# piljoong-jeong/nerf_meets_mlx

Measured on AMD Instinct MI355X. Metric: train+render rays/sec on Lego 800x800 (synthetic), coarse+fine 64+128, higher is better.
Workload: dtype split16 (fp16x2 render / bf16x2 train MFMA operands ~ 22 / 16 significand bits; fp32 accumulate)

## Files before the change

### nerf_meets_mlx_amd/csrc/mlp22.h

```cpp
#pragma once
#include <hip/hip_runtime.h>
#include <stdint.h>

namespace nerf {
namespace f22 {

constexpr int F_PAIRS = 1172, F_FRAGS = 2 * F_PAIRS, F_PADDED = 2368, BIAS_FLOATS = 2496;
constexpr int64_t PACKED_BYTES = (int64_t)F_PADDED * 1024 + (int64_t)BIAS_FLOATS * 4;

extern int g_tiles;
int pack(const float* params, void* packed22, hipStream_t s);
int forward(const void* packed22, const float* x, const float* rays, const float* z, int64_t M, int n, int freq_mode,
            float* out, int persistent_wgs, hipStream_t s);

}
}
```

### nerf_meets_mlx_amd/csrc/mlp22.hip

```cpp
#include "mlp_layout.h"
#include "mlp22.h"

#ifndef NERF_F22_SINF
#define NERF_F22_SINF 0
#endif

#ifndef NERF_F22_PIN
#define NERF_F22_PIN 1
#endif
#ifndef NERF_F22_AGPR
#define NERF_F22_AGPR 1
#endif
#ifndef NERF_F22_MIXSUB
#define NERF_F22_MIXSUB 1
#endif
#ifndef NERF_F22_RG3
#define NERF_F22_RG3 4
#endif
#ifndef NERF_F22_IGLP
#define NERF_F22_IGLP 0
#endif

namespace nerf {
namespace f22 {

typedef _Float16 h8 __attribute__((ext_vector_type(8)));
typedef _Float16 h2 __attribute__((ext_vector_type(2)));
typedef float f32x2 __attribute__((ext_vector_type(2)));
typedef unsigned int u32x4 __attribute__((ext_vector_type(4)));

constexpr float LO_SCALE = 2048.0f, LO_INV = 1.0f / 2048.0f;
constexpr float F16_MIN_NORMAL = 6.103515625e-05f;
constexpr int CHUNKS = F_PADDED / RING_CHUNK;
static_assert(CHUNKS * RING_CHUNK == F_PADDED && F_FRAGS % 4 == 0 && F_PAIRS == L::F16_TOTAL, "f22 stream layout");

struct HiLo { unsigned hi, lo; };
__device__ __forceinline__ HiLo split2(float v0, float v1) {
  const f32x2 v = {v0, v1};
  const h2 hh = __builtin_convertvector(v, h2);
#if NERF_F22_MIXSUB
  const f32x2 r = {__builtin_fmaf((float)hh[0], -LO_SCALE, v0 * LO_SCALE), __builtin_fmaf((float)hh[1], -LO_SCALE, v1 * LO_SCALE)};
#else
  const f32x2 r = {(v0 - (float)hh[0]) * LO_SCALE, (v1 - (float)hh[1]) * LO_SCALE};
#endif
  return HiLo{__builtin_bit_cast(unsigned, hh), __builtin_bit_cast(unsigned, __builtin_convertvector(r, h2))};
}

constexpr int PACK_THREADS = (F_PADDED / 2) * 64 + BIAS_FLOATS;
__global__ void __launch_bounds__(256) pack22_kernel(const float* __restrict__ p, u32x4* __restrict__ wf,
                                                     float* __restrict__ bias) {
  const int t = blockIdx.x * 256 + threadIdx.x;
  if (t < (F_PADDED / 2) * 64) {
    const int fp = t >> 6, lane = t & 63;
    u32x4 hi = {0u, 0u, 0u, 0u}, lo = {0u, 0u, 0u, 0u};
    if (fp < F_PAIRS) {
#pragma unroll
      for (int j = 0; j < 8; j += 2) {
        float w[2];
        _Float16 wh[2], wl[2];
#pragma unroll
        for (int e = 0; e < 2; ++e) {
          w[e] = fwd_src16(p, fp, lane & 15, lane >> 4, j + e);
          wh[e] = __builtin_fabsf(w[e]) < F16_MIN_NORMAL ? (_Float16)0.0f : (_Float16)w[e];
          wl[e] = (_Float16)((w[e] - (float)wh[e]) * LO_SCALE);
        }
        const h2 a = {wh[0], wh[1]}, b = {wl[0], wl[1]};
        hi[j >> 1] = __builtin_bit_cast(unsigned, a);
        lo[j >> 1] = __builtin_bit_cast(unsigned, b);
      }
    }
    wf[(2 * fp) * 64 + lane] = hi;
    wf[(2 * fp + 1) * 64 + lane] = lo;
  } else if (t < PACK_THREADS) {
    const int s = t - (F_PADDED / 2) * 64;
    float v = 0.0f;
    if (s < 2048) v = p[L::pb(s >> 8) + (s & 255)];
    else if (s < L::BI_ALPHA) v = p[L::P_BF + (s - L::BI_FEAT)];
    else if (s < L::BI_DIR) v = (s == L::BI_ALPHA) ? p[L::P_BA] : 0.0f;
    else if (s < L::BI_RGB) v = p[L::P_BD + (s - L::BI_DIR)];
    else v = (s - L::BI_RGB) < 3 ? p[L::P_BR + (s - L::BI_RGB)] : 0.0f;
    bias[s] = v;
  }
}

__device__ __forceinline__ float sin_acc(float x, float f, float ph) {
  const float a = x * f;
#if NERF_F22_SINF
  return ph != 0.0f ? cosf(a) : sinf(a);
#else
  const float k = __builtin_rintf(a * 0.15915494309189535f);
  float r = __builtin_fmaf(-k, 6.2831854820251465f, a);
  r = __builtin_fmaf(-k, -1.7484556000744487e-07f, r);
  return __builtin_amdgcn_sinf(__builtin_fmaf(r, 0.15915494309189535f, ph));
#endif
}

struct Pe22 { float fa, fb, fc, phc, fd; int g; };
__device__ __forceinline__ Pe22 pe22_setup(const PeFreq& fr, int g) {
  Pe22 q;
  q.fa = g == 0 ? fr.pos[0] : g == 1 ? fr.pos[2] : g == 2 ? fr.pos[4] : fr.pos[6];
  q.fb = g == 0 ? fr.pos[1] : g == 1 ? fr.pos[3] : g == 2 ? fr.pos[5] : fr.pos[7];
  q.fc = g < 2 ? fr.pos[8] : fr.pos[9];
  q.phc = (g & 1) ? 0.25f : 0.0f;
  q.fd = g == 0 ? fr.dir[0] : g == 1 ? fr.dir[1] : g == 2 ? fr.dir[2] : fr.dir[3];
  q.g = g;
  return q;
}

template <int COUNT>
__device__ __forceinline__ void split_slots(const float (&v)[COUNT], u32x4* hi, u32x4* lo) {
#pragma unroll
  for (int j = 0; j < COUNT; j += 2) {
    const HiLo q = split2(v[j], v[j + 1]);
    hi[j >> 3][(j & 7) >> 1] = q.hi; lo[j >> 3][(j & 7) >> 1] = q.lo;
  }
}

__device__ __forceinline__ void pe22_pos(const Pe22& q, const float (&p)[3], u32x4 (&peh)[2], u32x4 (&pel)[2]) {
  float v[16];
#pragma unroll
  for (int sl = 0; sl < 12; ++sl) v[sl] = sin_acc(p[sl % 3], sl < 6 ? q.fa : q.fb, (sl % 6) >= 3 ? 0.25f : 0.0f);
#pragma unroll
  for (int k = 0; k < 3; ++k) v[12 + k] = sin_acc(p[k], q.fc, q.phc);
  v[15] = q.g == 0 ? p[0] : q.g == 1 ? p[1] : q.g == 2 ? p[2] : 0.0f;
  split_slots<16>(v, peh, pel);
}
__device__ __forceinline__ void pe22_dir(const Pe22& q, const float (&d)[3], u32x4 (&dph)[1], u32x4 (&dpl)[1]) {
  float w[8];
#pragma unroll
  for (int j = 0; j < 6; ++j) w[j] = sin_acc(d[j % 3], q.fd, j >= 3 ? 0.25f : 0.0f);
  w[6] = q.g == 0 ? d[0] : q.g == 1 ? d[1] : q.g == 2 ? d[2] : 0.0f;
  w[7] = 0.0f;
  split_slots<8>(w, dph, dpl);
}
__device__ __forceinline__ void pe22_encode(const Pe22& q, const float (&p)[3], const float (&d)[3], u32x4 (&peh)[2],
                                            u32x4 (&pel)[2], u32x4 (&dph)[1], u32x4 (&dpl)[1]) {
  pe22_pos(q, p, peh, pel);
  pe22_dir(q, d, dph, dpl);
}
__device__ __forceinline__ void pe22_row(const float* __restrict__ row, int g, u32x4 (&peh)[2], u32x4 (&pel)[2],
                                         u32x4 (&dph)[1], u32x4 (&dpl)[1]) {
  float v[16], w[8];
#pragma unroll
  for (int sl = 0; sl < 16; ++sl) {
    const int ch = pos_chan16(sl >> 3, g, sl & 7);
    v[sl] = ch >= 0 ? row[ch] : 0.0f;
  }
#pragma unroll
  for (int j = 0; j < 8; ++j) {
    const int ch = dir_chan16(g, j);
    w[j] = ch >= 0 ? row[63 + ch] : 0.0f;
  }
  split_slots<16>(v, peh, pel);
  split_slots<8>(w, dph, dpl);
}

__device__ __forceinline__ f32x4 mfma16(const u32x4& a, const u32x4& b, const f32x4& c) {
#if NERF_ABLATE == 41 || NERF_ABLATE == 42
  return c;
#endif
  return __builtin_amdgcn_mfma_f32_16x16x32_f16(__builtin_bit_cast(h8, a), __builtin_bit_cast(h8, b), c, 0, 0, 0);
}

template <int NS, int KS, int NT, bool RELU, class WS, bool PARK_LDS = false>
__device__ __forceinline__ void layer22(WS& ws, int pbase, int bias_slot, const u32x4 (&ih)[NS][KS], const u32x4 (&il)[NS][KS],
                                        u32x4 (&oh)[NS][NT / 2], u32x4 (&ol)[NS][NT / 2], int lane, unsigned park_addr = 0u) {
  const int g = lane >> 4;
  f32x4 pm[NS], pc[NS];
  if (PARK_LDS) asm volatile("ds_write_b128 %0, %1" :: "v"(park_addr), "v"(il[NS - 1][KS - 1]) : "memory");
#if NERF_F22_IGLP >= 0
  __builtin_amdgcn_iglp_opt(NERF_F22_IGLP);
#endif
  constexpr int NP = 2 * NS;
  auto piece = [&](int nt, int pcs, f32x4 (&m)[NS], f32x4 (&c)[NS]) {
    const int s = pcs >> 1, i = 2 * (pcs & 1);
#if NERF_ABLATE == 41 || NERF_ABLATE == 42
    return;
#endif
#if NERF_F22_PIN
    if (pcs == 0) {
#pragma unroll
      for (int t = 0; t < NS; ++t) asm volatile("" : "+v"(m[t]), "+v"(c[t]));
    }
#endif
    float v0 = __builtin_fmaf(c[s][i], LO_INV, m[s][i]), v1 = __builtin_fmaf(c[s][i + 1], LO_INV, m[s][i + 1]);
    if (RELU) { v0 = __builtin_elementwise_maximum(v0, 0.0f); v1 = __builtin_elementwise_maximum(v1, 0.0f); }
    const HiLo q = split2(v0, v1);
    oh[s][nt >> 1][2 * (nt & 1) + (i >> 1)] = q.hi; ol[s][nt >> 1][2 * (nt & 1) + (i >> 1)] = q.lo;
#if NERF_F22_AGPR
    if ((nt & 1) && i == 2) asm volatile("" : "+a"(oh[s][nt >> 1]), "+a"(ol[s][nt >> 1]));
#endif
  };
  auto piece_at = [](int q) { return NS == 2 ? (KS >= 8 ? 1 + 2 * q : (q * KS) / 4) : (KS >= 8 ? 1 + (q * (KS - 1)) / NP : (q * KS) / NP); };
#pragma unroll
  for (int nt = 0; nt < NT; ++nt) {
    const float4 b = ws.bias4(bias_slot + 16 * nt + 4 * g);
    f32x4 m[NS], c[NS];
    m[0][0] = b.x; m[0][1] = b.y; m[0][2] = b.z; m[0][3] = b.w;
    c[0] = f32x4{0.0f, 0.0f, 0.0f, 0.0f};
#pragma unroll
    for (int t = 1; t < NS; ++t) { m[t] = m[0]; c[t] = c[0]; }
#pragma unroll
    for (int ks = 0; ks < KS; ++ks) {
      const int fp = pbase + nt * KS + ks;
      const u32x4 ah = __builtin_bit_cast(u32x4, next_frag(ws, 2 * fp, lane));
      const u32x4 al = __builtin_bit_cast(u32x4, next_frag(ws, 2 * fp + 1, lane));
      if (NS == 2) {
        m[0] = mfma16(ah, ih[0][ks], m[0]);
        c[0] = mfma16(ah, il[0][ks], c[0]);
        m[1] = mfma16(ah, ih[1][ks], m[1]);
        c[1] = mfma16(ah, il[1][ks], c[1]);
        c[0] = mfma16(al, ih[0][ks], c[0]);
        c[1] = mfma16(al, ih[1][ks], c[1]);
      } else {
#pragma unroll
        for (int t = 0; t < NS; ++t) {
          m[t] = mfma16(ah, ih[t][ks], m[t]);
          if (PARK_LDS && t == NS - 1 && ks == KS - 1) {
            u32x4 b;
            asm volatile("ds_read_b128 %0, %1\n\ts_waitcnt lgkmcnt(0)" : "=v"(b) : "v"(park_addr) : "memory");
            c[t] = mfma16(ah, b, c[t]);
          } else {
            c[t] = mfma16(ah, il[t][ks], c[t]);
          }
        }
#pragma unroll
        for (int t = 0; t < NS; ++t) c[t] = mfma16(al, ih[t][ks], c[t]);
      }
      if (nt > 0) {
#pragma unroll
        for (int q = 0; q < NP; ++q)
          if (piece_at(q) == ks) piece(nt - 1, q, pm, pc);
      }
    }
#pragma unroll
    for (int t = 0; t < NS; ++t) { pm[t] = m[t]; pc[t] = c[t]; }
  }
#pragma unroll
  for (int q = 0; q < NP; ++q) piece(NT - 1, q, pm, pc);
}

template <int NS, int KS, class WS>
__device__ __forceinline__ void head22(WS& ws, int pbase, int bias_slot, const u32x4 (&ih)[NS][KS], const u32x4 (&il)[NS][KS],
                                       f32x4 (&out)[NS], int lane) {
  const int g = lane >> 4;
  const float4 b = ws.bias4(bias_slot + 4 * g);
  f32x4 m[NS], c[NS];
  m[0][0] = b.x; m[0][1] = b.y; m[0][2] = b.z; m[0][3] = b.w;
  c[0] = f32x4{0.0f, 0.0f, 0.0f, 0.0f};
#pragma unroll
  for (int t = 1; t < NS; ++t) { m[t] = m[0]; c[t] = c[0]; }
#pragma unroll
  for (int ks = 0; ks < KS; ++ks) {
    const u32x4 ah = __builtin_bit_cast(u32x4, next_frag(ws, 2 * (pbase + ks), lane));
    const u32x4 al = __builtin_bit_cast(u32x4, next_frag(ws, 2 * (pbase + ks) + 1, lane));
    if (NS == 2) {
      m[0] = mfma16(ah, ih[0][ks], m[0]);
      c[0] = mfma16(ah, il[0][ks], c[0]);
      m[1] = mfma16(ah, ih[1][ks], m[1]);
      c[1] = mfma16(ah, il[1][ks], c[1]);
      c[0] = mfma16(al, ih[0][ks], c[0]);
      c[1] = mfma16(al, ih[1][ks], c[1]);
    } else {
#pragma unroll
      for (int t = 0; t < NS; ++t) { m[t] = mfma16(ah, ih[t][ks], m[t]); c[t] = mfma16(ah, il[t][ks], c[t]); }
#pragma unroll
      for (int t = 0; t < NS; ++t) c[t] = mfma16(al, ih[t][ks], c[t]);
    }
  }
#pragma unroll
  for (int s = 0; s < NS; ++s)
#pragma unroll
    for (int i = 0; i < 4; ++i) out[s][i] = __builtin_fmaf(c[s][i], LO_INV, m[s][i]);
}

constexpr int NW22 = 4, NW22_ = NW22;
constexpr int PARK_OFF = RING_LDS_BYTES;
template <int NS> constexpr int park_bytes() { return NS > 2 ? (6 * NS + 4) * 64 * NW22_ * 4 : 0; }
template <int K> __device__ __forceinline__ void lds_put(unsigned addr, float v) {
  asm volatile("ds_write_b32 %0, %1 offset:%2" :: "v"(addr), "v"(v), "i"(1024 * K) : "memory");
}
template <int K> __device__ __forceinline__ float lds_get(unsigned addr) {
  float v;
  asm volatile("ds_read_b32 %0, %1 offset:%2\n\ts_waitcnt lgkmcnt(0)" : "=v"(v) : "v"(addr), "i"(1024 * K) : "memory");
  return v;
}
template <int S> __device__ __forceinline__ void park_put(unsigned park, const float (&p)[3], const float (&d)[3]) {
  lds_put<6 * S + 0>(park, p[0]); lds_put<6 * S + 1>(park, p[1]); lds_put<6 * S + 2>(park, p[2]);
  lds_put<6 * S + 3>(park, d[0]); lds_put<6 * S + 4>(park, d[1]); lds_put<6 * S + 5>(park, d[2]);
}
template <int S, int OFF> __device__ __forceinline__ void park_get(unsigned park, float (&v)[3]) {
  v[0] = lds_get<6 * S + OFF>(park); v[1] = lds_get<6 * S + OFF + 1>(park); v[2] = lds_get<6 * S + OFF + 2>(park);
}
__device__ __forceinline__ void park_put_s(int s, unsigned park, const float (&p)[3], const float (&d)[3]) {
  if (s == 0) park_put<0>(park, p, d); else if (s == 1) park_put<1>(park, p, d); else park_put<2>(park, p, d);
}
template <int OFF> __device__ __forceinline__ void park_get_s(int s, unsigned park, float (&v)[3]) {
  if (s == 0) park_get<0, OFF>(park, v); else if (s == 1) park_get<1, OFF>(park, v); else park_get<2, OFF>(park, v);
}

template <int NS, int MODE, class WS>
__device__ __forceinline__ void tiles22(const FwdArgs& a, WS& ws, int64_t wtile0, int64_t nwtiles, int lane, PassQueue& pq) {
  constexpr bool RECOMP = NS > 2;
  static_assert(!RECOMP || MODE == 1, "the 48-sample form takes rays + depths");
  const int c = lane & 15, g = lane >> 4;
  u32x4 peh[NS][2], pel[NS][2], dph[NS][1], dpl[NS][1];
  const unsigned park = ws.lds0 + PARK_OFF + 4u * (unsigned)(ws.wv * 64 + lane);
  pq.ask(ws.wv, lane);
  const Pe22 q = pe22_setup(a.fr, g);
  {
    const int64_t wt = wtile0 < nwtiles ? wtile0 : nwtiles - 1;
#pragma unroll
    for (int s = 0; s < NS; ++s) {
      int64_t m = wt * (16 * NS) + 16 * s + c; if (m >= a.M) m = a.M - 1;
      if (MODE == 0) {
        pe22_row(a.x + m * 90, g, peh[s], pel[s], dph[s], dpl[s]);
      } else {
        const int64_t ray = (int64_t)((unsigned)m / (unsigned)a.n);
        const float* rr = a.rays + ray * NERF_RAY_STRIDE;
        float p[3], d[3];
#if NERF_ABLATE == 3
        (void)rr;
#pragma unroll
        for (int k = 0; k < 3; ++k) { p[k] = 0.001f * (float)(m & 1023) + (float)k; d[k] = 0.5f; }
#else
        const float zv = a.z[m];
#pragma unroll
        for (int k = 0; k < 3; ++k) { p[k] = rr[k] + zv * rr[3 + k]; d[k] = rr[8 + k]; }
#endif
        if (RECOMP) {
          park_put_s(s, park, p, d);
          pe22_pos(q, p, peh[s], pel[s]);
        } else {
          pe22_encode(q, p, d, peh[s], pel[s], dph[s], dpl[s]);
        }
      }
    }
  }
  pq.publish(ws.wv);
  u32x4 hah[NS][8], hal[NS][8], hbh[NS][8], hbl[NS][8];
  layer22<NS, 2, 16, true>(ws, L16::F_L0, 0, peh, pel, hah, hal, lane);
  layer22<NS, 8, 16, true>(ws, L16::F_L1 + 0 * 128, 256, hah, hal, hbh, hbl, lane);
  layer22<NS, 8, 16, true>(ws, L16::F_L1 + 1 * 128, 512, hbh, hbl, hah, hal, lane);
  layer22<NS, 8, 16, true>(ws, L16::F_L1 + 2 * 128, 768, hah, hal, hbh, hbl, lane);
  layer22<NS, 8, 16, true>(ws, L16::F_L1 + 3 * 128, 1024, hbh, hbl, hah, hal, lane);
  {
    u32x4 cth[NS][10], ctl[NS][10];
#pragma unroll
    for (int s = 0; s < NS; ++s) {
      if (RECOMP) {
        float pp[3];
        park_get_s<0>(s, park, pp);
        pe22_pos(q, pp, peh[s], pel[s]);
      }
      cth[s][0] = peh[s][0]; cth[s][1] = peh[s][1]; ctl[s][0] = pel[s][0]; ctl[s][1] = pel[s][1];
#pragma unroll
      for (int k = 0; k < 8; ++k) { cth[s][2 + k] = hah[s][k]; ctl[s][2 + k] = hal[s][k]; }
    }
    layer22<NS, 10, 16, true, WS, (NS > 2)>(ws, L16::F_L5, 1280, cth, ctl, hbh, hbl, lane,
                                            ws.lds0 + PARK_OFF + 6 * NS * 64 * NW22 * 4 + 16u * (unsigned)(ws.wv * 64 + lane));
  }
  layer22<NS, 8, 16, true>(ws, L16::F_L6, 1536, hbh, hbl, hah, hal, lane);
  layer22<NS, 8, 16, true>(ws, L16::F_L7, 1792, hah, hal, hbh, hbl, lane);
  layer22<NS, 8, 16, false>(ws, L16::F_FA, L::BI_FEAT, hbh, hbl, hah, hal, lane);
  f32x4 alpha[NS];
  head22<NS, 8>(ws, L16::F_FA + 128, L::BI_ALPHA, hbh, hbl, alpha, lane);
  u32x4 hdh[NS][4], hdl[NS][4];
  {
    u32x4 cth[NS][9], ctl[NS][9];
#pragma unroll
    for (int s = 0; s < NS; ++s) {
#pragma unroll
      for (int k = 0; k < 8; ++k) { cth[s][k] = hah[s][k]; ctl[s][k] = hal[s][k]; }
      if (RECOMP) {
        float dd[3];
        park_get_s<3>(s, park, dd);
        pe22_dir(q, dd, dph[s], dpl[s]);
      }
      cth[s][8] = dph[s][0]; ctl[s][8] = dpl[s][0];
    }
    layer22<NS, 9, 8, true>(ws, L16::F_DIR, L::BI_DIR, cth, ctl, hdh, hdl, lane);
  }
  f32x4 rgb[NS];
  head22<NS, 4>(ws, L16::F_RGB, L::BI_RGB, hdh, hdl, rgb, lane);
#pragma unroll
  for (int s = 0; s < NS; ++s) {
    const int64_t m = wtile0 * (16 * NS) + 16 * s + c;
    if (g == 0 && wtile0 < nwtiles && m < a.M) {
      float4 o; o.x = rgb[s][0]; o.y = rgb[s][1]; o.z = rgb[s][2]; o.w = alpha[s][0];
      *reinterpret_cast<float4*>(a.out + m * 4) = o;
    }
  }
}

template <int MODE, int NS = 2>
__global__ void __launch_bounds__(64 * NW22) mlp22_fwd_kernel(FwdArgs a) {
  const int lane = threadIdx.x & 63;
  const int wv = __builtin_amdgcn_readfirstlane(threadIdx.x >> 6);
  const int64_t nwtiles = (a.M + 16 * NS - 1) / (16 * NS), nsuper = (nwtiles + NW22 - 1) / NW22;
  NERF_STAMP2_DECL();
  RingW<CHUNKS, F_FRAGS, (NS > 2 ? NERF_F22_RG3 : 4), NW22, RING_CHUNK, RING_STAGES, true, true> ws;
  ws.wsrc = reinterpret_cast<const char*>(a.wf);
  ws.lane16 = 16 * lane;
  ws.lds0 = __builtin_amdgcn_readfirstlane(lds_addr_of(ring_smem));
  ws.wv = wv;
  ws.start(lane);
  ring_load_bias(a.bias, BIAS_FLOATS);
  __syncthreads();
  NERF_STAMP2_LOOP();
  PassQueue pq;
  pq.init(a.queue, ws.lds0 + RING_BIAS_OFF);
  for (int64_t sp = blockIdx.x; sp < nsuper;) {
    int ln = lane;
    asm volatile("" : "+v"(ln));
    ws.new_pass();
    tiles22<NS, MODE>(a, ws, sp * NW22 + wv, nwtiles, ln, pq);
    NERF_STAMP2_PASS();
    sp = pq.next(sp);
  }
  NERF_STAMP2_END();
  ws.drain();
  pq.leave();
}

int pack(const float* params, void* packed22, hipStream_t s) {
  char* base = static_cast<char*>(packed22);
  return launch<pack22_kernel>("nerf_mlp_pack (split-fp16 image)", dim3((PACK_THREADS + 255) / 256), dim3(256), 0, s, params,
                               reinterpret_cast<u32x4*>(base), reinterpret_cast<float*>(base + (size_t)F_PADDED * 1024));
}

int g_tiles = 0;

int forward(const void* packed22, const float* x, const float* rays, const float* z, int64_t M, int n, int freq_mode,
            float* out, int persistent_wgs, hipStream_t s) {
  FwdArgs a;
  a.queue = passq_slot();
  const char* base = static_cast<const char*>(packed22);
  a.wf = reinterpret_cast<const bf16x8*>(base);
  a.bias = reinterpret_cast<const float*>(base + (size_t)F_PADDED * 1024);
  a.x = x; a.rays = rays; a.z = z; a.M = M; a.n = n; a.out = out; a.acts = nullptr; a.astride = 0;
  fill_freqs(a.fr.pos, a.fr.dir, freq_mode);
  int tiles = g_tiles;
  if (tiles == 0) {
    const int64_t w = persistent_wgs > 0 ? persistent_wgs : 1;
    const int64_t p2 = (((M + 31) / 32 + NW22 - 1) / NW22 + w - 1) / w, p3 = (((M + 47) / 48 + NW22 - 1) / NW22 + w - 1) / w;
    tiles = 100 * p2 < 141 * p3 ? 2 : 3;
  }
  return with_index<3>(x ? 0 : (tiles == 3 ? 2 : 1), [&](auto form) {
    constexpr int MODE = decltype(form)::value == 0 ? 0 : 1, NS = decltype(form)::value == 2 ? 3 : 2;
    const int64_t nsuper = ((M + 16 * NS - 1) / (16 * NS) + NW22 - 1) / NW22;
    return launch<mlp22_fwd_kernel<MODE, NS>>("mlp forward (split fp16)", dim3(persistent_grid(nsuper, persistent_wgs)), dim3(64 * NW22),
                                             Lds(RING_LDS_BYTES + park_bytes<NS>(), RING_LDS_BYTES + park_bytes<3>()), s, a);
  });
}

}
}
NERF_STAMP2_EXPORT(nerf_debug_stamps2_mlp22)
```

### nerf_meets_mlx_amd/csrc/mlp_index.h

```cpp
#pragma once
#if !defined(__HIPCC__) && !defined(__host__)
#define __host__
#define __device__
#endif
#include "mlp_params.h"

namespace nerf {

namespace L {
constexpr int F_L0 = 0, F_L1 = 32, F_L5 = 544, F_L6 = 704, F_L7 = 832, F_FA = 960, F_DIR = 1104, F_RGB = 1176;
constexpr int F_TOTAL = 1184;
constexpr int B_RGB = 0, B_DIR = 4, B_FA = 68, B_L7 = 204, B_L6 = 332, B_L5 = 460, B_L4 = 588;
constexpr int B_TOTAL = 1100, B_PADDED = 1120;
}

__host__ __device__ constexpr int kperm(int ks, int h, int j) { return 16 * ks + 8 * (j >> 2) + 4 * h + (j & 3); }
__host__ __device__ constexpr int kperm_ks(int kk) { return kk >> 4; }
__host__ __device__ constexpr int kperm_h(int kk) { return (kk >> 2) & 1; }
__host__ __device__ constexpr int kperm_j(int kk) { return 4 * ((kk >> 3) & 1) + (kk & 3); }

__host__ __device__ constexpr int fwd_index(int f, int r, int h, int j) {
  if (f < L::F_L1) {
    const int nt = f / 4, ks = f % 4;
    const int kk = kperm(ks, h, j);
    return kk < 63 ? L::P_W0 + (32 * nt + r) * 63 + kk : -1;
  }
  if (f < L::F_L5) {
    const int l = 1 + (f - L::F_L1) / 128, g = (f - L::F_L1) % 128;
    const int nt = g / 16, ks = g % 16;
    return L::pw(l) + (32 * nt + r) * 256 + kperm(ks, h, j);
  }
  if (f < L::F_L6) {
    const int g = f - L::F_L5;
    const int nt = g / 20, ks = g % 20;
    const int kk = kperm(ks, h, j), n = 32 * nt + r;
    if (kk < 64) return kk < 63 ? L::P_W5 + n * 319 + kk : -1;
    return L::P_W5 + n * 319 + 63 + (kk - 64);
  }
  if (f < L::F_FA) {
    const int l = 6 + (f - L::F_L6) / 128, g = (f - L::F_L6) % 128;
    const int nt = g / 16, ks = g % 16;
    return L::pw(l) + (32 * nt + r) * 256 + kperm(ks, h, j);
  }
  if (f < L::F_DIR) {
    const int g = f - L::F_FA;
    const int nt = g / 16, ks = g % 16;
    const int kk = kperm(ks, h, j);
    if (nt < 8) return L::P_WF + (32 * nt + r) * 256 + kk;
    return r == 0 ? L::P_WA + kk : -1;
  }
  if (f < L::F_RGB) {
    const int g = f - L::F_DIR;
    const int nt = g / 18, ks = g % 18;
    const int kk = kperm(ks, h, j), n = 32 * nt + r;
    if (kk < 256) return L::P_WD + n * 283 + kk;
    return (kk - 256) < 27 ? L::P_WD + n * 283 + kk : -1;
  }
  const int ks = f - L::F_RGB;
  return r < 3 ? L::P_WR + r * 128 + kperm(ks, h, j) : -1;
}

__host__ __device__ constexpr int bwd_index(int f, int r, int h, int j) {
  if (f < L::B_DIR) {
    const int nn = kperm(0, h, j);
    return nn < 3 ? L::P_WR + nn * 128 + 32 * f + r : -1;
  }
  if (f < L::B_FA) {
    const int g = f - L::B_DIR, kt = g / 8, ns = g % 8;
    return L::P_WD + kperm(ns, h, j) * 283 + 32 * kt + r;
  }
  if (f < L::B_L7) {
    const int g = f - L::B_FA, kt = g / 17, ns = g % 17;
    const int nn = kperm(ns, h, j);
    if (ns < 16) return L::P_WF + nn * 256 + 32 * kt + r;
    return nn == 256 ? L::P_WA + 32 * kt + r : -1;
  }
  const int g = f - L::B_L7, li = g / 128, q = g % 128, kt = q / 16, ns = q % 16;
  const int l = 7 - li, nn = kperm(ns, h, j), row = 32 * kt + r;
  if (l == 5) return L::P_W5 + nn * 319 + 63 + row;
  return L::pw(l) + nn * 256 + row;
}

struct FragElem { int f, r, h, j; };
__host__ __device__ constexpr FragElem fwd_elem_feature(int row, int col) {
  return FragElem{L::F_FA + 16 * (row >> 5) + kperm_ks(col), row & 31, kperm_h(col), kperm_j(col)};
}
__host__ __device__ constexpr FragElem fwd_elem_dir0(int row, int col) {
  return FragElem{L::F_DIR + 18 * (row >> 5) + kperm_ks(col), row & 31, kperm_h(col), kperm_j(col)};
}
__host__ __device__ constexpr int frag_elem_offset(const FragElem& e) { return (e.f * 64 + 32 * e.h + e.r) * 8 + e.j; }

}
```

### nerf_meets_mlx_amd/csrc/mlp_layout.h

```cpp
#pragma once
#include "mlp_ring.h"
#include "mlp_params.h"
#include "mlp_index.h"

namespace nerf {

namespace L {

constexpr int BI_FEAT = 2048, BI_ALPHA = 2304, BI_DIR = 2336, BI_RGB = 2464, BI_TOTAL = 2496;
constexpr int F16_TOTAL = 1172, F16_PADDED = 1184;
constexpr int64_t F16_OFFSET = (int64_t)(F_TOTAL + B_PADDED) * 1024 + BI_TOTAL * 4;
constexpr int64_t PACKED_BYTES = F16_OFFSET + (int64_t)F16_PADDED * 1024;

constexpr int A_PE = 0, A_DPE = 4, A_H0 = 6;
constexpr int A_FEAT = 134, A_HD = 150;
constexpr int A_MASK = 158, A_SLOTS = 167;
constexpr int Z_L0 = 0;
constexpr int Z_F = 128, Z_A = 144, Z_D = 145, Z_RGB = 153, Z_SLOTS = 154;
}


namespace L16 {
constexpr int F_L0 = 0, F_L1 = 32, F_L5 = 544, F_L6 = 704, F_L7 = 832, F_FA = 960, F_DIR = 1096, F_RGB = 1168;
constexpr int CHUNKS = L::F16_PADDED / RING_CHUNK;
}
__host__ __device__ constexpr int kperm16(int ks, int g, int j) { return 32 * ks + 16 * (j >> 2) + 4 * g + (j & 3); }
__host__ __device__ constexpr int pos_chan16(int ks, int g, int j) {
  const int sl = 8 * ks + j;
  if (sl < 12) return 3 + 6 * (2 * g + sl / 6) + (sl % 6);
  if (sl < 15) return 3 + 6 * (8 + (g >> 1)) + 3 * (g & 1) + (sl - 12);
  return g < 3 ? g : -1;
}
__host__ __device__ constexpr int dir_chan16(int g, int j) {
  if (j < 6) return 3 + 6 * g + j;
  return (j == 6 && g < 3) ? g : -1;
}

__device__ inline float fwd_src16(const float* __restrict__ p, int f, int i, int g, int j) {
  if (f < L16::F_L1) {
    const int nt = f / 2, ch = pos_chan16(f % 2, g, j);
    return ch >= 0 ? p[L::P_W0 + (16 * nt + i) * 63 + ch] : 0.0f;
  }
  if (f < L16::F_L5) {
    const int q = f - L16::F_L1, l = 1 + q / 128, r = q % 128;
    return p[L::pw(l) + (16 * (r / 8) + i) * 256 + kperm16(r % 8, g, j)];
  }
  if (f < L16::F_L6) {
    const int q = f - L16::F_L5, n = 16 * (q / 10) + i, ks = q % 10;
    if (ks < 2) { const int ch = pos_chan16(ks, g, j); return ch >= 0 ? p[L::P_W5 + n * 319 + ch] : 0.0f; }
    return p[L::P_W5 + n * 319 + 63 + kperm16(ks - 2, g, j)];
  }
  if (f < L16::F_FA) {
    const int q = f - L16::F_L6, l = 6 + q / 128, r = q % 128;
    return p[L::pw(l) + (16 * (r / 8) + i) * 256 + kperm16(r % 8, g, j)];
  }
  if (f < L16::F_DIR) {
    const int q = f - L16::F_FA;
    if (q < 128) return p[L::P_WF + (16 * (q / 8) + i) * 256 + kperm16(q % 8, g, j)];
    return i == 0 ? p[L::P_WA + kperm16(q - 128, g, j)] : 0.0f;
  }
  if (f < L16::F_RGB) {
    const int q = f - L16::F_DIR, n = 16 * (q / 9) + i, ks = q % 9;
    if (ks < 8) return p[L::P_WD + n * 283 + kperm16(ks, g, j)];
    const int ch = dir_chan16(g, j);
    return ch >= 0 ? p[L::P_WD + n * 283 + 256 + ch] : 0.0f;
  }
  if (f < L::F16_TOTAL) return i < 3 ? p[L::P_WR + i * 128 + kperm16(f - L16::F_RGB, g, j)] : 0.0f;
  return 0.0f;
}


}
```

Baseline: 1.220 million.

## Fold linear feature layer into direction layer weights in f22 render path

The feature layer has no activation, so its weights and bias are folded into the direction layer during packing (W_dir·W_feat computed in double, bias folded likewise). The render kernel then skips the 256x256 feature layer and feeds the trunk output straight into the direction layer, removing about 128 fragment pairs of MFMA work and weight streaming per sample. Because of the register pressure this changes, a second parked input fragment is spilled to LDS in layer 5. The risk is that the folded product is less precise under the fp16 hi/lo split, and packing becomes more expensive.

Measured after the change: 1.305 million, median of 6. 1.07x the previous value.

```diff
diff --git a/nerf_meets_mlx_amd/csrc/mlp22.h b/nerf_meets_mlx_amd/csrc/mlp22.h
--- a/nerf_meets_mlx_amd/csrc/mlp22.h
+++ b/nerf_meets_mlx_amd/csrc/mlp22.h
@@ -1,17 +1,63 @@
 #pragma once
+#ifdef __HIPCC__
 #include <hip/hip_runtime.h>
+#endif
 #include <stdint.h>
+#include "mlp_index.h"
+
+#ifndef NERF_F22_FOLD
+#define NERF_F22_FOLD 1
+#endif
 
 namespace nerf {
 namespace f22 {
 
-constexpr int F_PAIRS = 1172, F_FRAGS = 2 * F_PAIRS, F_PADDED = 2368, BIAS_FLOATS = 2496;
+constexpr int P_L0 = 0, P_L1 = 32, P_L5 = 544, P_L6 = 704, P_L7 = 832, P_HEADS = 960;
+#if NERF_F22_FOLD
+constexpr int P_ALPHA = P_HEADS, P_DIR = P_ALPHA + 8, P_RGB = P_DIR + 72, F_PAIRS = P_RGB + 4;
+#else
+constexpr int P_FEAT = P_HEADS, P_ALPHA = P_FEAT + 128, P_DIR = P_ALPHA + 8, P_RGB = P_DIR + 72, F_PAIRS = P_RGB + 4;
+#endif
+constexpr int F_CHUNK = 32;
+constexpr int F_FRAGS = 2 * F_PAIRS, F_STREAM = (F_FRAGS + F_CHUNK - 1) / F_CHUNK * F_CHUNK, CHUNKS = F_STREAM / F_CHUNK;
+constexpr int F_PADDED = 2368, BIAS_FLOATS = 2496;
 constexpr int64_t PACKED_BYTES = (int64_t)F_PADDED * 1024 + (int64_t)BIAS_FLOATS * 4;
+static_assert(F_STREAM <= F_PADDED && F_FRAGS % 4 == 0, "f22 stream layout");
 
+#if NERF_F22_FOLD
+constexpr int SRC_ZERO = -1, SRC_FOLD = -2;
+struct Src { int p, n, k; };
+__host__ __device__ constexpr Src src_param(int p) { return Src{p, 0, 0}; }
+__host__ __device__ constexpr Src src_pos_chan(int row_base, int ks, int g, int j) {
+  return pos_chan16(ks, g, j) >= 0 ? src_param(row_base + pos_chan16(ks, g, j)) : Src{SRC_ZERO, 0, 0};
+}
+__host__ __device__ constexpr Src stream_src(int fp, int i, int g, int j) {
+  if (fp < P_L1) return src_pos_chan(L::P_W0 + (16 * (fp / 2) + i) * 63, fp % 2, g, j);
+  if (fp < P_L5 || (fp >= P_L6 && fp < P_HEADS)) {
+    const int q = fp < P_L5 ? fp - P_L1 : fp - P_L6, l = (fp < P_L5 ? 1 : 6) + q / 128, r = q % 128;
+    return src_param(L::pw(l) + (16 * (r / 8) + i) * 256 + kperm16(r % 8, g, j));
+  }
+  if (fp < P_L6) {
+    const int q = fp - P_L5, n = 16 * (q / 10) + i, ks = q % 10;
+    return ks < 2 ? src_pos_chan(L::P_W5 + n * 319, ks, g, j) : src_param(L::P_W5 + n * 319 + 63 + kperm16(ks - 2, g, j));
+  }
+  if (fp < P_DIR) return i == 0 ? src_param(L::P_WA + kperm16(fp - P_ALPHA, g, j)) : Src{SRC_ZERO, 0, 0};
+  if (fp < P_RGB) {
+    const int q = fp - P_DIR, n = 16 * (q / 9) + i, ks = q % 9;
+    if (ks < 8) return Src{SRC_FOLD, n, kperm16(ks, g, j)};
+    return dir_chan16(g, j) >= 0 ? src_param(L::P_WD + n * 283 + 256 + dir_chan16(g, j)) : Src{SRC_ZERO, 0, 0};
+  }
+  if (fp < F_PAIRS) return i < 3 ? src_param(L::P_WR + i * 128 + kperm16(fp - P_RGB, g, j)) : Src{SRC_ZERO, 0, 0};
+  return Src{SRC_ZERO, 0, 0};
+}
+#endif
+
+#ifdef __HIPCC__
 extern int g_tiles;
 int pack(const float* params, void* packed22, hipStream_t s);
 int forward(const void* packed22, const float* x, const float* rays, const float* z, int64_t M, int n, int freq_mode,
             float* out, int persistent_wgs, hipStream_t s);
+#endif
 
 }
 }
diff --git a/nerf_meets_mlx_amd/csrc/mlp22.hip b/nerf_meets_mlx_amd/csrc/mlp22.hip
--- a/nerf_meets_mlx_amd/csrc/mlp22.hip
+++ b/nerf_meets_mlx_amd/csrc/mlp22.hip
@@ -16,6 +16,9 @@
 #endif
 #ifndef NERF_F22_RG3
 #define NERF_F22_RG3 4
+#endif
+#ifndef NERF_F22_PARK
+#define NERF_F22_PARK (NERF_F22_FOLD ? 2 : 1)
 #endif
 #ifndef NERF_F22_IGLP
 #define NERF_F22_IGLP 0
@@ -31,8 +34,13 @@
 
 constexpr float LO_SCALE = 2048.0f, LO_INV = 1.0f / 2048.0f;
 constexpr float F16_MIN_NORMAL = 6.103515625e-05f;
-constexpr int CHUNKS = F_PADDED / RING_CHUNK;
-static_assert(CHUNKS * RING_CHUNK == F_PADDED && F_FRAGS % 4 == 0 && F_PAIRS == L::F16_TOTAL, "f22 stream layout");
+static_assert(F_CHUNK == RING_CHUNK && CHUNKS == (F_FRAGS + RING_CHUNK - 1) / RING_CHUNK && CHUNKS * RING_CHUNK <= F_PADDED, "f22 ring chunks");
+static_assert(P_L0 == L16::F_L0 && P_L1 == L16::F_L1 && P_L5 == L16::F_L5 && P_L6 == L16::F_L6 && P_L7 == L16::F_L7 && P_HEADS == L16::F_FA, "f22 trunk");
+#if NERF_F22_FOLD
+static_assert(F_PAIRS == L::F16_TOTAL - 128 && CHUNKS == 66 && F_FRAGS % RING_CHUNK == (2 * L::F16_TOTAL) % RING_CHUNK, "f22 folded stream");
+#else
+static_assert(F_PAIRS == L::F16_TOTAL && P_ALPHA == L16::F_FA + 128 && P_DIR == L16::F_DIR && P_RGB == L16::F_RGB && CHUNKS == 74, "f22 stream layout");
+#endif
 
 struct HiLo { unsigned hi, lo; };
 __device__ __forceinline__ HiLo split2(float v0, float v1) {
@@ -54,13 +62,34 @@
     const int fp = t >> 6, lane = t & 63;
     u32x4 hi = {0u, 0u, 0u, 0u}, lo = {0u, 0u, 0u, 0u};
     if (fp < F_PAIRS) {
+#if NERF_F22_FOLD
+      float fold[8] = {0.0f, 0.0f, 0.0f, 0.0f, 0.0f, 0.0f, 0.0f, 0.0f};
+      if (fp >= P_DIR && fp < P_RGB && (fp - P_DIR) % 9 < 8) {
+        const float* __restrict__ wd = p + L::P_WD + (16 * ((fp - P_DIR) / 9) + (lane & 15)) * 283;
+        const float* __restrict__ wfk = p + L::P_WF + kperm16((fp - P_DIR) % 9, lane >> 4, 0);
+        double acc[8] = {0.0, 0.0, 0.0, 0.0, 0.0, 0.0, 0.0, 0.0};
+#pragma unroll 4
+        for (int f = 0; f < 256; ++f) {
+          const double a = (double)wd[f];
+#pragma unroll
+          for (int e = 0; e < 8; ++e) acc[e] = __builtin_fma(a, (double)wfk[f * 256 + 16 * (e >> 2) + (e & 3)], acc[e]);
+        }
+#pragma unroll
+        for (int e = 0; e < 8; ++e) fold[e] = (float)acc[e];
+      }
+#endif
 #pragma unroll
       for (int j = 0; j < 8; j += 2) {
         float w[2];
         _Float16 wh[2], wl[2];
 #pragma unroll
         for (int e = 0; e < 2; ++e) {
+#if NERF_F22_FOLD
+          const Src src = stream_src(fp, lane & 15, lane >> 4, j + e);
+          w[e] = src.p >= 0 ? p[src.p] : src.p == SRC_FOLD ? fold[j + e] : 0.0f;
+#else
           w[e] = fwd_src16(p, fp, lane & 15, lane >> 4, j + e);
+#endif
           wh[e] = __builtin_fabsf(w[e]) < F16_MIN_NORMAL ? (_Float16)0.0f : (_Float16)w[e];
           wl[e] = (_Float16)((w[e] - (float)wh[e]) * LO_SCALE);
         }
@@ -75,9 +104,20 @@
     const int s = t - (F_PADDED / 2) * 64;
     float v = 0.0f;
     if (s < 2048) v = p[L::pb(s >> 8) + (s & 255)];
+#if NERF_F22_FOLD
+    else if (s < L::BI_ALPHA) v = 0.0f;
+    else if (s < L::BI_DIR) v = (s == L::BI_ALPHA) ? p[L::P_BA] : 0.0f;
+    else if (s < L::BI_RGB) {
+      const float* __restrict__ wd = p + L::P_WD + (s - L::BI_DIR) * 283;
+      double acc = 0.0;
+      for (int f = 0; f < 256; ++f) acc = __builtin_fma((double)wd[f], (double)p[L::P_BF + f], acc);
+      v = (float)(acc + (double)p[L::P_BD + (s - L::BI_DIR)]);
+    }
+#else
     else if (s < L::BI_ALPHA) v = p[L::P_BF + (s - L::BI_FEAT)];
     else if (s < L::BI_DIR) v = (s == L::BI_ALPHA) ? p[L::P_BA] : 0.0f;
     else if (s < L::BI_RGB) v = p[L::P_BD + (s - L::BI_DIR)];
+#endif
     else v = (s - L::BI_RGB) < 3 ? p[L::P_BR + (s - L::BI_RGB)] : 0.0f;
     bias[s] = v;
   }
@@ -162,12 +202,15 @@
   return __builtin_amdgcn_mfma_f32_16x16x32_f16(__builtin_bit_cast(h8, a), __builtin_bit_cast(h8, b), c, 0, 0, 0);
 }
 
-template <int NS, int KS, int NT, bool RELU, class WS, bool PARK_LDS = false>
+template <int NS, int KS, int NT, bool RELU, class WS, int PARK_LDS = 0>
 __device__ __forceinline__ void layer22(WS& ws, int pbase, int bias_slot, const u32x4 (&ih)[NS][KS], const u32x4 (&il)[NS][KS],
-                                        u32x4 (&oh)[NS][NT / 2], u32x4 (&ol)[NS][NT / 2], int lane, unsigned park_addr = 0u) {
+                                        u32x4 (&oh)[NS][NT / 2], u32x4 (&ol)[NS][NT / 2], int lane, unsigned park_addr = 0u, unsigned park2_addr = 0u) {
   const int g = lane >> 4;
   f32x4 pm[NS], pc[NS];
   if (PARK_LDS) asm volatile("ds_write_b128 %0, %1" :: "v"(park_addr), "v"(il[NS - 1][KS - 1]) : "memory");
+  if (PARK_LDS >= 2)
+    asm volatile("ds_write_b32 %0, %1\n\tds_write_b32 %0, %2 offset:1024\n\tds_write_b32 %0, %3 offset:2048\n\tds_write_b32 %0, %4 offset:6144"
+                 :: "v"(park2_addr), "v"(il[NS - 2][KS - 1][0]), "v"(il[NS - 2][KS - 1][1]), "v"(il[NS - 2][KS - 1][2]), "v"(il[NS - 2][KS - 1][3]) : "memory");
 #if NERF_F22_IGLP >= 0
   __builtin_amdgcn_iglp_opt(NERF_F22_IGLP);
 #endif
@@ -220,6 +263,11 @@
             u32x4 b;
             asm volatile("ds_read_b128 %0, %1\n\ts_waitcnt lgkmcnt(0)" : "=v"(b) : "v"(park_addr) : "memory");
             c[t] = mfma16(ah, b, c[t]);
+          } else if (PARK_LDS >= 2 && t == NS - 2 && ks == KS - 1) {
+            u32x4 b;
+            asm volatile("ds_read_b32 %0, %4\n\tds_read_b32 %1, %4 offset:1024\n\tds_read_b32 %2, %4 offset:2048\n\tds_read_b32 %3, %4 offset:6144\n\ts_waitcnt lgkmcnt(0)"
+                         : "=&v"(b[0]), "=&v"(b[1]), "=&v"(b[2]), "=&v"(b[3]) : "v"(park2_addr) : "memory");
+            c[t] = mfma16(ah, b, c[t]);
           } else {
             c[t] = mfma16(ah, il[t][ks], c[t]);
           }
@@ -357,21 +405,26 @@
 #pragma unroll
       for (int k = 0; k < 8; ++k) { cth[s][2 + k] = hah[s][k]; ctl[s][2 + k] = hal[s][k]; }
     }
-    layer22<NS, 10, 16, true, WS, (NS > 2)>(ws, L16::F_L5, 1280, cth, ctl, hbh, hbl, lane,
-                                            ws.lds0 + PARK_OFF + 6 * NS * 64 * NW22 * 4 + 16u * (unsigned)(ws.wv * 64 + lane));
+    layer22<NS, 10, 16, true, WS, (NS > 2 ? NERF_F22_PARK : 0)>(ws, L16::F_L5, 1280, cth, ctl, hbh, hbl, lane,
+                                            ws.lds0 + PARK_OFF + 6 * NS * 64 * NW22 * 4 + 16u * (unsigned)(ws.wv * 64 + lane), park);
   }
   layer22<NS, 8, 16, true>(ws, L16::F_L6, 1536, hbh, hbl, hah, hal, lane);
   layer22<NS, 8, 16, true>(ws, L16::F_L7, 1792, hah, hal, hbh, hbl, lane);
-  layer22<NS, 8, 16, false>(ws, L16::F_FA, L::BI_FEAT, hbh, hbl, hah, hal, lane);
+#if NERF_F22_FOLD
+  u32x4 (&fth)[NS][8] = hbh, (&ftl)[NS][8] = hbl;
+#else
+  layer22<NS, 8, 16, false>(ws, P_FEAT, L::BI_FEAT, hbh, hbl, hah, hal, lane);
+  u32x4 (&fth)[NS][8] = hah, (&ftl)[NS][8] = hal;
+#endif
   f32x4 alpha[NS];
-  head22<NS, 8>(ws, L16::F_FA + 128, L::BI_ALPHA, hbh, hbl, alpha, lane);
+  head22<NS, 8>(ws, P_ALPHA, L::BI_ALPHA, hbh, hbl, alpha, lane);
   u32x4 hdh[NS][4], hdl[NS][4];
   {
     u32x4 cth[NS][9], ctl[NS][9];
 #pragma unroll
     for (int s = 0; s < NS; ++s) {
 #pragma unroll
-      for (int k = 0; k < 8; ++k) { cth[s][k] = hah[s][k]; ctl[s][k] = hal[s][k]; }
+      for (int k = 0; k < 8; ++k) { cth[s][k] = fth[s][k]; ctl[s][k] = ftl[s][k]; }
       if (RECOMP) {
         float dd[3];
         park_get_s<3>(s, park, dd);
@@ -379,10 +432,10 @@
       }
       cth[s][8] = dph[s][0]; ctl[s][8] = dpl[s][0];
     }
-    layer22<NS, 9, 8, true>(ws, L16::F_DIR, L::BI_DIR, cth, ctl, hdh, hdl, lane);
+    layer22<NS, 9, 8, true>(ws, P_DIR, L::BI_DIR, cth, ctl, hdh, hdl, lane);
   }
   f32x4 rgb[NS];
-  head22<NS, 4>(ws, L16::F_RGB, L::BI_RGB, hdh, hdl, rgb, lane);
+  head22<NS, 4>(ws, P_RGB, L::BI_RGB, hdh, hdl, rgb, lane);
 #pragma unroll
   for (int s = 0; s < NS; ++s) {
     const int64_t m = wtile0 * (16 * NS) + 16 * s + c;
diff --git a/nerf_meets_mlx_amd/csrc/mlp_index.h b/nerf_meets_mlx_amd/csrc/mlp_index.h
--- a/nerf_meets_mlx_amd/csrc/mlp_index.h
+++ b/nerf_meets_mlx_amd/csrc/mlp_index.h
@@ -18,6 +18,18 @@
 __host__ __device__ constexpr int kperm_ks(int kk) { return kk >> 4; }
 __host__ __device__ constexpr int kperm_h(int kk) { return (kk >> 2) & 1; }
 __host__ __device__ constexpr int kperm_j(int kk) { return 4 * ((kk >> 3) & 1) + (kk & 3); }
+
+__host__ __device__ constexpr int kperm16(int ks, int g, int j) { return 32 * ks + 16 * (j >> 2) + 4 * g + (j & 3); }
+__host__ __device__ constexpr int pos_chan16(int ks, int g, int j) {
+  const int sl = 8 * ks + j;
+  if (sl < 12) return 3 + 6 * (2 * g + sl / 6) + (sl % 6);
+  if (sl < 15) return 3 + 6 * (8 + (g >> 1)) + 3 * (g & 1) + (sl - 12);
+  return g < 3 ? g : -1;
+}
+__host__ __device__ constexpr int dir_chan16(int g, int j) {
+  if (j < 6) return 3 + 6 * g + j;
+  return (j == 6 && g < 3) ? g : -1;
+}
 
 __host__ __device__ constexpr int fwd_index(int f, int r, int h, int j) {
   if (f < L::F_L1) {
diff --git a/nerf_meets_mlx_amd/csrc/mlp_layout.h b/nerf_meets_mlx_amd/csrc/mlp_layout.h
--- a/nerf_meets_mlx_amd/csrc/mlp_layout.h
+++ b/nerf_meets_mlx_amd/csrc/mlp_layout.h
@@ -23,17 +23,6 @@
 namespace L16 {
 constexpr int F_L0 = 0, F_L1 = 32, F_L5 = 544, F_L6 = 704, F_L7 = 832, F_FA = 960, F_DIR = 1096, F_RGB = 1168;
 constexpr int CHUNKS = L::F16_PADDED / RING_CHUNK;
-}
-__host__ __device__ constexpr int kperm16(int ks, int g, int j) { return 32 * ks + 16 * (j >> 2) + 4 * g + (j & 3); }
-__host__ __device__ constexpr int pos_chan16(int ks, int g, int j) {
-  const int sl = 8 * ks + j;
-  if (sl < 12) return 3 + 6 * (2 * g + sl / 6) + (sl % 6);
-  if (sl < 15) return 3 + 6 * (8 + (g >> 1)) + 3 * (g & 1) + (sl - 12);
-  return g < 3 ? g : -1;
-}
-__host__ __device__ constexpr int dir_chan16(int g, int j) {
-  if (j < 6) return 3 + 6 * g + j;
-  return (j == 6 && g < 3) ? g : -1;
 }
 
 __device__ inline float fwd_src16(const float* __restrict__ p, int f, int i, int g, int j) {
```
